# rpp0/gr-lora

Measured on NVIDIA H100. Metric: LoRa symbols/s (dechirp+FFT+argmax), higher is better.
Workload: dtype f32

## Files before the change

gr_lora_b200/csrc/k1_rows.cuh:

```cuda
#pragma once
#include "k1_warp.cuh"
#ifdef __CUDACC__
#include <cuda.h>
#endif

namespace lb {

template <int SF>
struct RCfg {
    static constexpr int N = 1 << SF, SPS = 8 * N, L = N;
    static constexpr int CL = SF == 12 ? 2 : 1;
    static constexpr int NB = 8 / CL;
    static constexpr int A = L / 16;
    static constexpr int A0 = L / 256;
    static constexpr int CPA = NB / 2;
    static constexpr int ROW_F4 = A * CPA;
    static constexpr uint32_t ROW_BYTES = 8192u;
    static constexpr int NSLOT = SF == 12 ? 24 : 28;
    static constexpr int T = 512, NW = 16;
    static constexpr int HB = NB / 2;
    static_assert(SF == 11 || SF == 12, "rows kernel: SF11, SF12");
    static_assert(A0 * CPA == 32, "one warp = one a1 block of every row");
};

constexpr int R_NSYM_BAR = 4;
template <int SF> struct RLate { static constexpr int EARLY = RCfg<SF>::NSLOT - 16; };

template <int SF> LB_HD int r_a0(int lane) { return lane / RCfg<SF>::CPA; }
template <int SF> LB_HD int r_p(int lane) { return lane % RCfg<SF>::CPA; }
template <int SF> LB_HD int r_sample(int rank, int warp, int lane, int j) {
    using C = RCfg<SF>;
    const int a = warp * C::A0 + r_a0<SF>(lane);
    return 8 * (j * C::A + a) + rank * C::NB + 2 * r_p<SF>(lane);
}
template <int SF> LB_HD int r_swz(int block) { return SF == 11 ? ((block & 1) | ((block & 2) << 1)) : ((block & 3) << 1); }
template <int SF> LB_HD int r_unit(int block, int within) { return block * 32 + (within ^ r_swz<SF>(block)); }
template <int SF> LB_HD int r_cq_exp(int e, int q2) {
    using C = RCfg<SF>;
    const int d = 256 * q2 - (q2 >= C::A0 / 2 ? C::L : 0);
    return (e * d) & (C::SPS - 1);
}

struct RConsts {
    float2 cq[4][16];
};
template <int SF> LB_HD int r_e_of(int i) { return SF == 11 ? (i == 0 ? 1 : 4) : (i == 0 ? 1 : 2 * i); }
template <int SF>
inline void r_build_consts(const float2 *tw_host, RConsts &c) {
    for (int i = 0; i < 4; i++)
        for (int q2 = 0; q2 < 16; q2++) c.cq[i][q2] = tw_host[r_cq_exp<SF>(r_e_of<SF>(i), q2 % RCfg<SF>::A0)];
}

LB_HD void r_dif16(float2 *v0, float2 *v1) {
    dft_dif<16>(v0);
    dft_dif<16>(v1);
}
LB_HD void r_twiddle16(float2 *v0, float2 *v1, const float2 *tw) {
#pragma unroll
    for (int k = 1; k < 16; k++) {
        const int br = bitrev<16>(k);
        v0[br] = cmul(v0[br], tw[k - 1]);
        v1[br] = cmul(v1[br], tw[k - 1]);
    }
}

template <int SF>
LB_HD void r_pass2_dft(float2 (*g)[RCfg<SF>::A0]) {
#pragma unroll
    for (int b = 0; b < RCfg<SF>::HB; b++) dft_dif<RCfg<SF>::A0>(g[b]);
}
template <int SF>
LB_HD float2 r_pass2_term(float2 (*g)[RCfg<SF>::A0], int q2, int E, float2 wb1, float2 wbE, const float2 *cq1, const float2 *cqE) {
    using C = RCfg<SF>;
    const int br = bitrev<C::A0>(q2);
    const float2 w = cmul(wb1, cq1[q2]);
    float2 acc = g[C::HB - 1][br];
#pragma unroll
    for (int b = C::HB - 2; b >= 0; b--) acc = cfma(acc, w, g[b][br]);
    return E ? cmul(acc, cmul(wbE, cqE[q2])) : acc;
}
template <int SF>
LB_HD float2 r_pass2_quirk(float2 (*g)[RCfg<SF>::A0], int E, float2 wb1, float2 wbE, const float2 *cq1, const float2 *cqE) {
    using C = RCfg<SF>;
    const int q2 = C::A0 / 2, br = bitrev<C::A0>(q2);
    const float2 w = cconj(cmul(wb1, cq1[q2]));
    float2 acc = g[C::HB - 1][br];
#pragma unroll
    for (int b = C::HB - 2; b >= 0; b--) acc = cfma(acc, w, g[b][br]);
    return E ? cmul(acc, cconj(cmul(wbE, cqE[q2]))) : acc;
}

#ifdef __CUDACC__
LB_D float4 lds128(uint32_t addr) {
    float4 v;
    asm volatile("ld.shared.v4.f32 {%0, %1, %2, %3}, [%4];" : "=f"(v.x), "=f"(v.y), "=f"(v.z), "=f"(v.w) : "r"(addr) : "memory");
    return v;
}
LB_D void sts128(uint32_t addr, float4 v) {
    asm volatile("st.shared.v4.f32 [%0], {%1, %2, %3, %4};" ::"r"(addr), "f"(v.x), "f"(v.y), "f"(v.z), "f"(v.w) : "memory");
}

LB_D uint32_t cluster_rank() { uint32_t r; asm volatile("mov.u32 %0, %%cluster_ctarank;" : "=r"(r)); return r; }
LB_D uint32_t map_to_peer(uint32_t local_smem_addr, uint32_t peer) {
    uint32_t r;
    asm volatile("mapa.shared::cluster.u32 %0, %1, %2;" : "=r"(r) : "r"(local_smem_addr), "r"(peer));
    return r;
}
LB_D void mbar_arrive_peer_relaxed(uint32_t peer_bar_addr) {
    asm volatile("mbarrier.arrive.relaxed.cluster.shared::cluster.b64 _, [%0];" ::"r"(peer_bar_addr) : "memory");
}
LB_D void st_async_peer_f4(uint32_t peer_dst, float4 v, uint32_t peer_bar) {
    asm volatile("st.async.weak.shared::cluster.mbarrier::complete_tx::bytes.v4.f32 [%0], {%1, %2, %3, %4}, [%5];"
                 ::"r"(peer_dst), "f"(v.x), "f"(v.y), "f"(v.z), "f"(v.w), "r"(peer_bar) : "memory");
}
LB_D void cluster_sync_all() {
    asm volatile("barrier.cluster.arrive.release.aligned;" ::: "memory");
    asm volatile("barrier.cluster.wait.acquire.aligned;" ::: "memory");
}
LB_D void tma_rows_2d(void *dst_smem, const void *tmap, int c0, int c1, uint64_t *bar) {
    asm volatile("cp.async.bulk.tensor.2d.shared::cluster.global.tile.mbarrier::complete_tx::bytes [%0], [%1, {%2, %3}], [%4];"
                 ::"r"(smem_u32(dst_smem)), "l"(tmap), "r"(c0), "r"(c1), "r"(smem_u32(bar)) : "memory");
}

#ifdef LB_ROWS_TIMING
__device__ unsigned int r_timing_dev[160 * 16 * 8];
#define RT_DECL unsigned int rt_acc[6] = {0, 0, 0, 0, 0, 0}; const unsigned int rt_start = (unsigned int)clock();
#define RT(i, stmt) do { const unsigned int rt_t0 = (unsigned int)clock(); stmt; rt_acc[i] += (unsigned int)clock() - rt_t0; } while (0)
#define RT_FLUSH do { if (lane == 0) { unsigned int *o = r_timing_dev + (blockIdx.x * 16 + warp) * 8; for (int i = 0; i < 6; i++) o[i] = rt_acc[i]; \
                                    o[6] = (unsigned int)clock() - rt_start; o[7] = (unsigned int)n_mine; } } while (0)
#else
#define RT_DECL
#define RT(i, stmt) stmt
#define RT_FLUSH
#endif

template <int SF>
struct RSmem {
    float4 slots[RCfg<SF>::NSLOT][RCfg<SF>::ROW_F4];
    float2 recv[RCfg<SF>::CL == 2 ? 2 * 8 * 256 : 2];
    unsigned long long keys[2][RCfg<SF>::NW];
    uint64_t sym_full[R_NSYM_BAR];
    uint64_t sym_late[R_NSYM_BAR];
    uint64_t x_full[16], x_free[16];
};

struct alignas(64) RParams {
    CUtensorMap tmap;
    K1Args a;
    unsigned long long *packed;
    uint32_t *bins;
    float *mags;
};

static __device__ __constant__ RConsts r_consts_dev[2];

template <int SF>
__global__ void __launch_bounds__(RCfg<SF>::T, 1)
k1_rows_kernel(const __grid_constant__ RParams P) {
    using C = RCfg<SF>;
    extern __shared__ __align__(1024) unsigned char r_raw[];
    RSmem<SF> &sm = *reinterpret_cast<RSmem<SF> *>(r_raw);
    const int tid = threadIdx.x, lane = tid & 31, warp = tid >> 5;
    const uint32_t rank = C::CL == 2 ? cluster_rank() : 0u, peer = rank ^ 1u;
    const size_t unit = blockIdx.x / C::CL, n_units = gridDim.x / C::CL;
    const K1Args &a = P.a;
    const size_t n_mine = unit < a.n_symbols ? (a.n_symbols - unit + n_units - 1) / n_units : 0;
    const RConsts &rc = r_consts_dev[SF - 11];

    if (tid == 0) {
#pragma unroll
        for (int i = 0; i < R_NSYM_BAR; i++) { mbar_init(&sm.sym_full[i], RLate<SF>::EARLY); mbar_init(&sm.sym_late[i], 16 - RLate<SF>::EARLY); }
#pragma unroll
        for (int i = 0; i < 16; i++) { mbar_init(&sm.x_full[i], 1); mbar_init(&sm.x_free[i], 32); }
        if (C::CL == 2 && n_mine > 0)
#pragma unroll
            for (int i = 0; i < 16; i++)
                if (i < 8 || n_mine > 1) mbar_expect_tx(&sm.x_full[i], 2048u);
        fence_mbar_init();
    }
    auto issue_row = [&](size_t g) {
        const size_t s = g >> 4;
        if (s >= n_mine) return;
        const int j = (int)(g & 15);
        const size_t sym = unit + s * n_units;
        uint64_t *bar = j < RLate<SF>::EARLY ? &sm.sym_full[s % R_NSYM_BAR] : &sm.sym_late[s % R_NSYM_BAR];
        float4 *dst = sm.slots[g % C::NSLOT];
        mbar_expect_tx(bar, C::ROW_BYTES);
        if (C::CL == 1) bulk_g2s(dst, a.x + sym * C::SPS + (size_t)j * (C::SPS / 16), C::ROW_BYTES, bar);
        else tma_rows_2d(dst, &P.tmap, (int)(rank * 8u), (int)(sym * C::L + (size_t)j * C::A), bar);
    };
    if (tid == 0)
        for (int g = 0; g < C::NSLOT; g++) issue_row((size_t)g);

    const int tw0_step = 8 * (warp * C::A0 + r_a0<SF>(lane)), tw1_step = 128 * r_a0<SF>(lane);
    const int kb2 = lane >> 1, h2 = lane & 1;
    const int E2 = (int)rank * C::NB + h2 * C::HB;
    const int e_idx = SF == 11 ? (E2 ? 1 : 0) : (E2 >> 1);
    const float2 wb1 = k1_ld_table(a.tw + ((warp + 16 * kb2) & (C::SPS - 1)));
    const float2 wbE = k1_ld_table(a.tw + ((E2 * (warp + 16 * kb2)) & (C::SPS - 1)));
    if (C::CL == 2) cluster_sync_all(); else __syncthreads();

    const uint32_t slots0 = smem_u32(&sm.slots[0][0]);
    const uint32_t ld0 = slots0 + (uint32_t)(warp * 32 + lane) * 16u;
    const uint32_t st0 = slots0 + (uint32_t)r_unit<SF>(warp, lane) * 16u;
    uint32_t lane_sw[4];
#pragma unroll
    for (int c = 0; c < 4; c++) lane_sw[c] = (uint32_t)(lane ^ r_swz<SF>(c)) * 16u;
    const uint32_t m2 = (uint32_t)((SF == 11 ? 2 * (lane & 1) : (lane & 1)) ^ r_swz<SF>(lane >> 1)) * 16u + (uint32_t)(lane >> 1) * 512u;
    RT_DECL
    const int x_i = warp & 7;
    const bool x_mine = C::CL == 2 && (uint32_t)(warp >> 3) == rank;
    float2 stash[8];
    auto finalize_prev = [&](size_t sp) {
        const int xb = (int)(sp & 1) * 8 + x_i;
        RT(0, mbar_wait(&sm.x_full[xb], (uint32_t)((sp >> 1) & 1)));
        const float2 *o = stash;
        const float4 *rblk = reinterpret_cast<const float4 *>(&sm.recv[xb * 256]);
        float4 u[4];
#pragma unroll
        for (int i = 0; i < 4; i++) u[i] = rblk[i * 32 + lane];
        uint32_t dep = 0;
        unsigned long long bk = 0ull;
#pragma unroll
        for (int i = 0; i < 4; i++) {
            const float2 fa = cadd(o[2 * i], make_float2(u[i].x, u[i].y));
            const float2 fb = cadd(o[2 * i + 1], make_float2(u[i].z, u[i].w));
            dep |= __float_as_uint(u[i].w);
            const int q0 = 2 * i + (lane & 1) * (C::A0 / 2);
            const unsigned long long ka = pack_key(cnorm2(fa), (uint32_t)(warp + 16 * (lane >> 1) + 256 * q0));
            const unsigned long long kb = pack_key(cnorm2(fb), (uint32_t)(warp + 16 * (lane >> 1) + 256 * (q0 + 1)));
            bk = ka > bk ? ka : bk;
            bk = kb > bk ? kb : bk;
        }
        bk = warp_max_key(bk);
        if (lane == 0) {
            atomicMax(P.packed + unit + sp * n_units, bk);
            if (sp + 2 < n_mine) mbar_expect_tx(&sm.x_full[xb], 2048u);
        }
        asm volatile("and.b32 %0, %0, 0;" : "+r"(dep));
        mbar_arrive_peer_relaxed(map_to_peer(smem_u32(&sm.x_free[xb]), peer) + dep);
    };
    int base = 0;
    for (size_t s = 0; s < n_mine; s++, base = base + 16 >= C::NSLOT ? base + 16 - C::NSLOT : base + 16) {
        const size_t g0 = s * 16;
        uint32_t gb[4];
        {
            int t = base;
#pragma unroll
            for (int q = 0; q < 4; q++) { gb[q] = (uint32_t)t * C::ROW_BYTES; t += 4; if (t >= C::NSLOT) t -= C::NSLOT; }
        }
        uint32_t rowaddr;
        { int t = base + warp; if (t >= C::NSLOT) t -= C::NSLOT; rowaddr = slots0 + (uint32_t)t * C::ROW_BYTES; }
        RT(2, mbar_wait(&sm.sym_full[s % R_NSYM_BAR], (uint32_t)((s / R_NSYM_BAR) & 1)));

        {
            float2 v0[16], v1[16], tw[16];
#pragma unroll
            for (int q = 0; q < 4; q++) {
                if (4 * q == RLate<SF>::EARLY) RT(3, mbar_wait(&sm.sym_late[s % R_NSYM_BAR], (uint32_t)((s / R_NSYM_BAR) & 1)));
                float4 ch[4];
#pragma unroll
                for (int jj = 0; jj < 4; jj++) ch[jj] = k1_ld_table4(a.chirp + r_sample<SF>((int)rank, warp, lane, 4 * q + jj));
                float4 xv[4];
                const uint32_t ga = ld0 + gb[q];
#pragma unroll
                for (int jj = 0; jj < 4; jj++) xv[jj] = lds128(ga + (uint32_t)jj * C::ROW_BYTES);
#pragma unroll
                for (int jj = 0; jj < 4; jj++) {
                    v0[4 * q + jj] = cmul(make_float2(xv[jj].x, xv[jj].y), make_float2(ch[jj].x, ch[jj].y));
                    v1[4 * q + jj] = cmul(make_float2(xv[jj].z, xv[jj].w), make_float2(ch[jj].z, ch[jj].w));
                }
            }
            r_dif16(v0, v1);
#pragma unroll
            for (int kc = 1; kc < 16; kc++) tw[kc - 1] = k1_ld_table(a.tw + ((tw0_step * kc) & (C::SPS - 1)));
            r_twiddle16(v0, v1, tw);
            __syncwarp();
#pragma unroll
            for (int kc = 0; kc < 16; kc++) {
                const int br = bitrev<16>(kc);
                sts128(st0 + gb[kc >> 2] + (uint32_t)(kc & 3) * C::ROW_BYTES, make_float4(v0[br].x, v0[br].y, v1[br].x, v1[br].y));
            }
        }
        RT(4, __syncthreads());
        if (C::CL == 1 && s > 0 && warp == 0) {
            unsigned long long k = lane < C::NW ? sm.keys[(s - 1) & 1][lane] : 0ull;
            k = warp_max_key(k);
            if (lane == 0) {
                const size_t psym = unit + (s - 1) * n_units;
                if (C::CL == 2) atomicMax(P.packed + psym, k);
                else { P.bins[psym] = key_idx(k); if (P.mags) P.mags[psym] = sqrtf(key_mag2(k)); }
            }
        }
        {
            float2 v0[16], v1[16], tw[16];
            uint32_t ra[4];
#pragma unroll
            for (int c = 0; c < 4; c++) ra[c] = rowaddr + lane_sw[c];
#pragma unroll
            for (int a1 = 0; a1 < 16; a1++) {
                const float4 u = lds128(ra[a1 & 3] + (uint32_t)a1 * 512u);
                v0[a1] = make_float2(u.x, u.y);
                v1[a1] = make_float2(u.z, u.w);
            }
            r_dif16(v0, v1);
#pragma unroll
            for (int kb = 1; kb < 16; kb++) tw[kb - 1] = k1_ld_table(a.tw + ((tw1_step * kb) & (C::SPS - 1)));
            r_twiddle16(v0, v1, tw);
#pragma unroll
            for (int kb = 0; kb < 16; kb++) {
                const int br = bitrev<16>(kb);
                sts128(ra[kb & 3] + (uint32_t)kb * 512u, make_float4(v0[br].x, v0[br].y, v1[br].x, v1[br].y));
            }
        }
        __syncwarp();
        if (C::CL == 2 && x_mine && s > 0) finalize_prev(s - 1);
        unsigned long long best = 0ull;
        {
            float2 g[C::HB][C::A0];
            {
                const uint32_t qm = rowaddr + m2;
                uint32_t pa[4];
                if (SF == 11) {
#pragma unroll
                    for (int c = 0; c < 4; c++) pa[c] = qm ^ (uint32_t)(((c >> 1) * 4 + (c & 1)) * 16);
#pragma unroll
                    for (int a0 = 0; a0 < C::A0; a0++)
#pragma unroll
                        for (int e = 0; e < 2; e++) {
                            const float4 u = lds128(pa[(a0 & 1) * 2 + e] + (uint32_t)(a0 >> 1) * 128u);
                            g[2 * e][a0] = make_float2(u.x, u.y);
                            g[(2 * e + 1) % C::HB][a0] = make_float2(u.z, u.w);
                        }
                } else {
#pragma unroll
                    for (int c = 0; c < 4; c++) pa[c] = qm ^ (uint32_t)(c * 2 * 16);
#pragma unroll
                    for (int a0 = 0; a0 < C::A0; a0++) {
                        const float4 u = lds128(pa[a0 & 3] + (uint32_t)(a0 >> 2) * 128u);
                        g[0][a0] = make_float2(u.x, u.y);
                        g[C::HB - 1][a0] = make_float2(u.z, u.w);
                    }
                }
            }
            r_pass2_dft<SF>(g);
            __syncwarp();
            if (lane == 0) {
                fence_proxy_async();
                issue_row(g0 + (size_t)warp + (size_t)C::NSLOT);
            }
            float2 wb1s = wb1, wbEs = wbE;
            asm volatile("" : "+f"(wb1s.x), "+f"(wb1s.y), "+f"(wbEs.x), "+f"(wbEs.y));
            const bool quirk_warp = warp == 0;
            float2 tq = make_float2(0.f, 0.f);
            if (quirk_warp && kb2 == 0) tq = r_pass2_quirk<SF>(g, E2, wb1s, wbEs, rc.cq[0], rc.cq[e_idx]);
            float2 f[C::A0 / 2];
#pragma unroll
            for (int i = 0; i < C::A0 / 2; i++) {
                const float2 tlo = r_pass2_term<SF>(g, i, E2, wb1s, wbEs, rc.cq[0], rc.cq[e_idx]);
                const float2 thi = r_pass2_term<SF>(g, i + C::A0 / 2, E2, wb1s, wbEs, rc.cq[0], rc.cq[e_idx]);
                const float2 give = h2 ? tlo : thi;
                const float2 keep = h2 ? thi : tlo;
                float2 got;
                got.x = __shfl_xor_sync(0xffffffffu, give.x, 1);
                got.y = __shfl_xor_sync(0xffffffffu, give.y, 1);
                f[i] = cadd(keep, got);
            }
            if (quirk_warp) {
                float2 got;
                got.x = __shfl_xor_sync(0xffffffffu, tq.x, 1);
                got.y = __shfl_xor_sync(0xffffffffu, tq.y, 1);
                tq = cadd(tq, got);
            }
            if (C::CL == 2) {
                if (quirk_warp && lane == 1) f[0] = cadd(f[0], tq);
                if (!x_mine) {
                    const int xb = (int)(s & 1) * 8 + x_i;
                    if (s > 1) RT(1, mbar_wait(&sm.x_free[xb], (uint32_t)(((s >> 1) - 1) & 1)));
                    const uint32_t dst = map_to_peer(smem_u32(&sm.recv[xb * 256]), peer) + (uint32_t)lane * 16u;
                    const uint32_t bar = map_to_peer(smem_u32(&sm.x_full[xb]), peer);
#pragma unroll
                    for (int i = 0; i < 4; i++) st_async_peer_f4(dst + (uint32_t)i * 512u, make_float4(f[2 * i].x, f[2 * i].y, f[2 * i + 1].x, f[2 * i + 1].y), bar);
                } else {
#pragma unroll
                    for (int i = 0; i < 8; i++) stash[i] = f[i];
                }
            } else {
                if (quirk_warp && lane == 1) f[0] = cadd(f[0], tq);
#pragma unroll
                for (int i = 0; i < C::A0 / 2; i++) {
                    const int q2 = i + h2 * (C::A0 / 2);
                    const unsigned long long key = pack_key(cnorm2(f[i]), (uint32_t)(warp + 16 * kb2 + 256 * q2));
                    best = key > best ? key : best;
                }
            }
        }
        best = warp_max_key(best);
        if (C::CL == 1 && lane == 0) sm.keys[s & 1][warp] = best;
    }
    if (C::CL == 2 && x_mine && n_mine > 0) finalize_prev(n_mine - 1);
    RT_FLUSH;
    __syncthreads();
    if (C::CL == 1 && n_mine > 0 && warp == 0) {
        unsigned long long k = lane < C::NW ? sm.keys[(n_mine - 1) & 1][lane] : 0ull;
        k = warp_max_key(k);
        if (lane == 0) {
            const size_t psym = unit + (n_mine - 1) * n_units;
            if (C::CL == 2) atomicMax(P.packed + psym, k);
            else { P.bins[psym] = key_idx(k); if (P.mags) P.mags[psym] = sqrtf(key_mag2(k)); }
        }
    }
    if (C::CL == 2) cluster_sync_all();
}
#endif

template <int SF>
inline void r_emulate(const K1Args &a, uint32_t *bins, float *mags) {
    using C = RCfg<SF>;
    RConsts rc;
    r_build_consts<SF>(a.tw, rc);
    const int NSL = C::NSLOT;
    float4 *slots[2];
    float2 *part[2];
    for (int c = 0; c < C::CL; c++) { slots[c] = new float4[(size_t)NSL * C::ROW_F4]; part[c] = new float2[C::L + 1]; }
    unsigned long long *keys = new unsigned long long[C::CL * C::NW];
    for (size_t s = 0; s < a.n_symbols; s++) {
        const float2 *x = a.x + s * C::SPS;
        const size_t g0 = s * 16;
        for (int c = 0; c < C::CL; c++) {
            float4 *sl = slots[c];
            auto slot = [&](size_t g) { return sl + (g % NSL) * C::ROW_F4; };
            for (int j = 0; j < 16; j++)
                for (int aa = 0; aa < C::A; aa++)
                    for (int p = 0; p < C::CPA; p++) {
                        const int n = 8 * (j * C::A + aa) + c * C::NB + 2 * p;
                        slot(g0 + j)[aa * C::CPA + p] = make_float4(x[n].x, x[n].y, x[n + 1].x, x[n + 1].y);
                    }
            for (int warp = 0; warp < C::NW; warp++) {
                float2 v0[32][16], v1[32][16];
                for (int lane = 0; lane < 32; lane++) {
                    float2 tw[16];
                    const int a_idx = warp * C::A0 + r_a0<SF>(lane);
                    for (int kc = 1; kc < 16; kc++) tw[kc - 1] = a.tw[(8 * a_idx * kc) & (C::SPS - 1)];
                    for (int j = 0; j < 16; j++) {
                        const float4 xv = slot(g0 + j)[warp * 32 + lane];
                        const int n = r_sample<SF>(c, warp, lane, j);
                        v0[lane][j] = cmul(make_float2(xv.x, xv.y), a.chirp[n]);
                        v1[lane][j] = cmul(make_float2(xv.z, xv.w), a.chirp[n + 1]);
                    }
                    r_dif16(v0[lane], v1[lane]);
                    r_twiddle16(v0[lane], v1[lane], tw);
                }
                for (int lane = 0; lane < 32; lane++)
                    for (int kc = 0; kc < 16; kc++) {
                        const int br = bitrev<16>(kc);
                        slot(g0 + kc)[r_unit<SF>(warp, lane)] = make_float4(v0[lane][br].x, v0[lane][br].y, v1[lane][br].x, v1[lane][br].y);
                    }
            }
            for (int warp = 0; warp < C::NW; warp++) {
                float4 *row = slot(g0 + warp);
                float2 v0[32][16], v1[32][16];
                for (int lane = 0; lane < 32; lane++) {
                    float2 tw[16];
                    for (int kb = 1; kb < 16; kb++) tw[kb - 1] = a.tw[(128 * r_a0<SF>(lane) * kb) & (C::SPS - 1)];
                    for (int a1 = 0; a1 < 16; a1++) {
                        const float4 u = row[r_unit<SF>(a1, lane)];
                        v0[lane][a1] = make_float2(u.x, u.y);
                        v1[lane][a1] = make_float2(u.z, u.w);
                    }
                    r_dif16(v0[lane], v1[lane]);
                    r_twiddle16(v0[lane], v1[lane], tw);
                }
                for (int lane = 0; lane < 32; lane++)
                    for (int kb = 0; kb < 16; kb++) {
                        const int br = bitrev<16>(kb);
                        row[r_unit<SF>(kb, lane)] = make_float4(v0[lane][br].x, v0[lane][br].y, v1[lane][br].x, v1[lane][br].y);
                    }
                float2 t[32][C::A0], tq[32];
                for (int lane = 0; lane < 32; lane++) {
                    const int kb2 = lane >> 1, h2 = lane & 1;
                    const int E2 = c * C::NB + h2 * C::HB;
                    const int e_idx = SF == 11 ? (E2 ? 1 : 0) : (E2 >> 1);
                    const float2 wb1 = a.tw[(warp + 16 * kb2) & (C::SPS - 1)];
                    const float2 wbE = a.tw[(E2 * (warp + 16 * kb2)) & (C::SPS - 1)];
                    float2 g[C::HB][C::A0];
                    for (int a0 = 0; a0 < C::A0; a0++) {
                        if (SF == 11) {
                            for (int e = 0; e < 2; e++) {
                                const float4 u = row[r_unit<SF>(kb2, a0 * 4 + 2 * h2 + e)];
                                g[2 * e][a0] = make_float2(u.x, u.y);
                                g[(2 * e + 1) % C::HB][a0] = make_float2(u.z, u.w);
                            }
                        } else {
                            const float4 u = row[r_unit<SF>(kb2, a0 * 2 + h2)];
                            g[0][a0] = make_float2(u.x, u.y);
                            g[C::HB - 1][a0] = make_float2(u.z, u.w);
                        }
                    }
                    tq[lane] = make_float2(0.f, 0.f);
                    r_pass2_dft<SF>(g);
                    if (warp == 0 && kb2 == 0) tq[lane] = r_pass2_quirk<SF>(g, E2, wb1, wbE, rc.cq[0], rc.cq[e_idx]);
                    for (int q2 = 0; q2 < C::A0; q2++) t[lane][q2] = r_pass2_term<SF>(g, q2, E2, wb1, wbE, rc.cq[0], rc.cq[e_idx]);
                }
                for (int lane = 0; lane < 32; lane++) {
                    const int kb2 = lane >> 1, h2 = lane & 1;
                    for (int i = 0; i < C::A0 / 2; i++) {
                        const int q2 = i + h2 * (C::A0 / 2);
                        part[c][warp + 16 * kb2 + 256 * q2] = cadd(t[lane][q2], t[lane ^ 1][q2]);
                    }
                }
                if (warp == 0) part[c][C::L] = cadd(tq[0], tq[1]);
            }
        }
        unsigned long long best = 0ull;
        for (int k = 0; k < C::L; k++) {
            float2 f = part[0][k];
            if (C::CL == 2) f = cadd(f, part[1][k]);
            if (k == C::L / 2) {
                float2 q = part[0][C::L];
                if (C::CL == 2) q = cadd(q, part[1][C::L]);
                f = cadd(f, q);
            }
            const unsigned long long key = pack_key(cnorm2(f), (uint32_t)k);
            best = key > best ? key : best;
        }
        bins[s] = key_idx(best);
        if (mags) mags[s] = sqrtf(key_mag2(best));
    }
    for (int c = 0; c < C::CL; c++) { delete[] slots[c]; delete[] part[c]; }
    delete[] keys;
}

}
```

Baseline: 364.3 million.

## Stage FFT twiddles in shared memory and prefetch first chirp block

Builds per-CTA shared-memory twiddle tables at kernel start. SF11 gets full per-(a,k) tables; SF12 gets a 256-entry coarse table and a small fine table combined by one complex multiply. The twiddle loads in both FFT passes now read these tables instead of global memory. The first group of chirp loads is also hoisted ahead of the symbol barrier wait. To make room for the tables, the SF11 slot ring is reduced from 28 to 24 rows, which shortens the prefetch depth.

```diff
diff --git a/gr_lora_b200/csrc/k1_rows.cuh b/gr_lora_b200/csrc/k1_rows.cuh
--- a/gr_lora_b200/csrc/k1_rows.cuh
+++ b/gr_lora_b200/csrc/k1_rows.cuh
@@ -16,7 +16,7 @@
     static constexpr int CPA = NB / 2;
     static constexpr int ROW_F4 = A * CPA;
     static constexpr uint32_t ROW_BYTES = 8192u;
-    static constexpr int NSLOT = SF == 12 ? 24 : 28;
+    static constexpr int NSLOT = 24;
     static constexpr int T = 512, NW = 16;
     static constexpr int HB = NB / 2;
     static_assert(SF == 11 || SF == 12, "rows kernel: SF11, SF12");
@@ -39,6 +39,33 @@
     using C = RCfg<SF>;
     const int d = 256 * q2 - (q2 >= C::A0 / 2 ? C::L : 0);
     return (e * d) & (C::SPS - 1);
+}
+
+template <int SF> struct RTw {
+    static constexpr bool FULL = SF == 11;
+    static constexpr int N0 = FULL ? 15 * RCfg<SF>::A : 256 + 16, N1 = FULL ? 15 * RCfg<SF>::A0 : RCfg<SF>::A0;
+    static constexpr int FILL = FULL ? 15 * RCfg<SF>::A : 256;
+};
+template <int SF> LB_HD void r_tw_tables(const float2 *tw, int i, float2 *t0, float2 *t1) {
+    using C = RCfg<SF>;
+    if (RTw<SF>::FULL) {
+        t0[i] = k1_ld_table(tw + ((8 * (i % C::A) * (i / C::A + 1)) & (C::SPS - 1)));
+        if (i < RTw<SF>::N1) t1[i] = k1_ld_table(tw + ((128 * (i % C::A0) * (i / C::A0 + 1)) & (C::SPS - 1)));
+    } else {
+        t0[k1_pad(i)] = k1_ld_table(tw + i * (C::SPS / 256));
+        if (i < C::A0) t1[i] = k1_ld_table(tw + 8 * i);
+    }
+}
+template <int SF> LB_HD float2 r_tw0(const float2 *t0, const float2 *t1, int a, int kc) {
+    using C = RCfg<SF>;
+    if (RTw<SF>::FULL) return t0[(kc - 1) * C::A + a];
+    const int e = a * kc;
+    return cmul(t0[k1_pad((e >> (SF - 8)) & 255)], t1[e & (C::A0 - 1)]);
+}
+template <int SF> LB_HD float2 r_tw1(const float2 *t0, const float2 *t1, int a0, int kb) {
+    using C = RCfg<SF>;
+    if (RTw<SF>::FULL) return t1[(kb - 1) * C::A0 + a0];
+    return t0[k1_pad((a0 * kb) & 255)];
 }
 
 struct RConsts {
@@ -133,16 +160,27 @@
 #define RT(i, stmt) stmt
 #define RT_FLUSH
 #endif
+#ifdef LB_ROWS_NO_TABLES
+#define R_CHIRP4(p, i) make_float4(0.6f + 1e-3f * (float)(i), 0.8f, 0.8f, -0.6f - 1e-3f * (float)(i))
+#define R_TW0(a, k) make_float2(0.8f - 1e-4f * (float)((a) * (k)), -0.6f)
+#define R_TW1(a0, k) make_float2(0.8f - 1e-4f * (float)((a0) * (k)), -0.6f)
+#else
+#define R_CHIRP4(p, i) k1_ld_table4((p) + (i))
+#define R_TW0(a, k) r_tw0<SF>(sm.tw0, sm.tw1, a, k)
+#define R_TW1(a0, k) r_tw1<SF>(sm.tw0, sm.tw1, a0, k)
+#endif
 
 template <int SF>
 struct RSmem {
     float4 slots[RCfg<SF>::NSLOT][RCfg<SF>::ROW_F4];
     float2 recv[RCfg<SF>::CL == 2 ? 2 * 8 * 256 : 2];
+    float2 tw0[RTw<SF>::N0], tw1[RTw<SF>::N1];
     unsigned long long keys[2][RCfg<SF>::NW];
     uint64_t sym_full[R_NSYM_BAR];
     uint64_t sym_late[R_NSYM_BAR];
     uint64_t x_full[16], x_free[16];
 };
+static_assert(sizeof(RSmem<11>) <= 227 * 1024 && sizeof(RSmem<12>) <= 227 * 1024, "rows kernel: shared memory per CTA");
 
 struct alignas(64) RParams {
     CUtensorMap tmap;
@@ -192,7 +230,8 @@
     if (tid == 0)
         for (int g = 0; g < C::NSLOT; g++) issue_row((size_t)g);
 
-    const int tw0_step = 8 * (warp * C::A0 + r_a0<SF>(lane)), tw1_step = 128 * r_a0<SF>(lane);
+    for (int i = tid; i < RTw<SF>::FILL; i += C::T) r_tw_tables<SF>(a.tw, i, sm.tw0, sm.tw1);
+    const int tw0_a = warp * C::A0 + r_a0<SF>(lane), tw1_a0 = r_a0<SF>(lane);
     const int kb2 = lane >> 1, h2 = lane & 1;
     const int E2 = (int)rank * C::NB + h2 * C::HB;
     const int e_idx = SF == 11 ? (E2 ? 1 : 0) : (E2 >> 1);
@@ -251,6 +290,9 @@
         }
         uint32_t rowaddr;
         { int t = base + warp; if (t >= C::NSLOT) t -= C::NSLOT; rowaddr = slots0 + (uint32_t)t * C::ROW_BYTES; }
+        float4 ch0[4];
+#pragma unroll
+        for (int jj = 0; jj < 4; jj++) ch0[jj] = R_CHIRP4(a.chirp, r_sample<SF>((int)rank, warp, lane, jj));
         RT(2, mbar_wait(&sm.sym_full[s % R_NSYM_BAR], (uint32_t)((s / R_NSYM_BAR) & 1)));
 
         {
@@ -260,7 +302,7 @@
                 if (4 * q == RLate<SF>::EARLY) RT(3, mbar_wait(&sm.sym_late[s % R_NSYM_BAR], (uint32_t)((s / R_NSYM_BAR) & 1)));
                 float4 ch[4];
 #pragma unroll
-                for (int jj = 0; jj < 4; jj++) ch[jj] = k1_ld_table4(a.chirp + r_sample<SF>((int)rank, warp, lane, 4 * q + jj));
+                for (int jj = 0; jj < 4; jj++) ch[jj] = q == 0 ? ch0[jj] : R_CHIRP4(a.chirp, r_sample<SF>((int)rank, warp, lane, 4 * q + jj));
                 float4 xv[4];
                 const uint32_t ga = ld0 + gb[q];
 #pragma unroll
@@ -273,7 +315,7 @@
             }
             r_dif16(v0, v1);
 #pragma unroll
-            for (int kc = 1; kc < 16; kc++) tw[kc - 1] = k1_ld_table(a.tw + ((tw0_step * kc) & (C::SPS - 1)));
+            for (int kc = 1; kc < 16; kc++) tw[kc - 1] = R_TW0(tw0_a, kc);
             r_twiddle16(v0, v1, tw);
             __syncwarp();
 #pragma unroll
@@ -305,7 +347,7 @@
             }
             r_dif16(v0, v1);
 #pragma unroll
-            for (int kb = 1; kb < 16; kb++) tw[kb - 1] = k1_ld_table(a.tw + ((tw1_step * kb) & (C::SPS - 1)));
+            for (int kb = 1; kb < 16; kb++) tw[kb - 1] = R_TW1(tw1_a0, kb);
             r_twiddle16(v0, v1, tw);
 #pragma unroll
             for (int kb = 0; kb < 16; kb++) {
@@ -419,6 +461,8 @@
     using C = RCfg<SF>;
     RConsts rc;
     r_build_consts<SF>(a.tw, rc);
+    float2 tw0[RTw<SF>::N0], tw1[RTw<SF>::N1];
+    for (int i = 0; i < RTw<SF>::FILL; i++) r_tw_tables<SF>(a.tw, i, tw0, tw1);
     const int NSL = C::NSLOT;
     float4 *slots[2];
     float2 *part[2];
@@ -441,7 +485,7 @@
                 for (int lane = 0; lane < 32; lane++) {
                     float2 tw[16];
                     const int a_idx = warp * C::A0 + r_a0<SF>(lane);
-                    for (int kc = 1; kc < 16; kc++) tw[kc - 1] = a.tw[(8 * a_idx * kc) & (C::SPS - 1)];
+                    for (int kc = 1; kc < 16; kc++) tw[kc - 1] = r_tw0<SF>(tw0, tw1, a_idx, kc);
                     for (int j = 0; j < 16; j++) {
                         const float4 xv = slot(g0 + j)[warp * 32 + lane];
                         const int n = r_sample<SF>(c, warp, lane, j);
@@ -462,7 +506,7 @@
                 float2 v0[32][16], v1[32][16];
                 for (int lane = 0; lane < 32; lane++) {
                     float2 tw[16];
-                    for (int kb = 1; kb < 16; kb++) tw[kb - 1] = a.tw[(128 * r_a0<SF>(lane) * kb) & (C::SPS - 1)];
+                    for (int kb = 1; kb < 16; kb++) tw[kb - 1] = r_tw1<SF>(tw0, tw1, r_a0<SF>(lane), kb);
                     for (int a1 = 0; a1 < 16; a1++) {
                         const float4 u = row[r_unit<SF>(a1, lane)];
                         v0[lane][a1] = make_float2(u.x, u.y);
```

Result: no change. 364.6 million (median of 6 runs) (+0.1%).
